# starlingonearth/MASt3R-SLAM-Quality-dualTSDF

Measured on AMD Instinct MI355X. Metric: SLAM frames/sec (infer+match+TSDF+GN) @512x384, higher is better.
Workload: dtype bf16

## Files before the change

include/mslam_hip.h:

```cpp
#ifndef MSLAM_HIP_H
#define MSLAM_HIP_H

#include <stddef.h>
#include <stdint.h>

#ifdef __cplusplus
extern "C" {
#endif

#define MSLAM_OK 0
#define MSLAM_EINVAL (-1)
#define MSLAM_EHIP (-2)
#define MSLAM_ENOMEM (-3)
#define MSLAM_ENODEV (-4)

const char* mslam_last_error(void);
int mslam_abi_version(void);
int mslam_device_check(void);


int mslam_iter_proj(const float* rays_img_with_grad, const float* pts_3d_norm,
                    const float* p_init, float* p_new, uint8_t* converged, int b, int h, int w,
                    int n, int max_iter, float lambda_init, float cost_thresh, void* stream);

int mslam_refine_matches(const uint16_t* D11, const uint16_t* D21, const int64_t* p1,
                         int64_t* p1_new, int b, int h, int w, int n, int fdim, int radius,
                         int dilation_max, void* stream);

int mslam_prep_iter_proj(const float* X11, const float* X21, const int64_t* idx_init,
                         float* rays_img_with_grad, float* pts_3d_norm, float* p_init, int b, int h,
                         int w, void* stream);

int mslam_match_occlusion(const float* X11, const float* X21, const float* p, int64_t* p1,
                          uint8_t* valid, int b, int h, int w, float dist_thresh, void* stream);

int mslam_pixel_to_lin(const int64_t* p1, int64_t* idx, int b, int n, int w, void* stream);

size_t mslam_gn_workspace_bytes(int num_poses, int num_edges, int num_points, int local_edges);

int mslam_gauss_newton_rays(float* Twc, const float* Xs, const float* Cs, const int64_t* ii,
                            const int64_t* jj, const int64_t* idx_ii2jj, const uint8_t* valid_match,
                            const float* Q, int num_poses, int num_points, int num_edges,
                            float sigma_ray, float sigma_dist, float C_thresh, float Q_thresh,
                            int max_iter, float delta_thresh, float* dx, void* workspace,
                            size_t workspace_bytes, void* stream);

int mslam_gauss_newton_calib(float* Twc, const float* Xs, const float* Cs, const float* K,
                             const int64_t* ii, const int64_t* jj, const int64_t* idx_ii2jj,
                             const uint8_t* valid_match, const float* Q, int num_poses, int num_points,
                             int num_edges, int height, int width, int pixel_border, float z_eps,
                             float sigma_pixel, float sigma_depth, float C_thresh, float Q_thresh,
                             int max_iter, float delta_thresh, float* dx, void* workspace,
                             size_t workspace_bytes, void* stream);

int mslam_gauss_newton_points(float* Twc, const float* Xs, const float* Cs, const int64_t* ii,
                              const int64_t* jj, const int64_t* idx_ii2jj, const uint8_t* valid_match,
                              const float* Q, int num_poses, int num_points, int num_edges,
                              float sigma_point, float C_thresh, float Q_thresh, int max_iter,
                              float delta_thresh, float* dx, void* workspace, size_t workspace_bytes,
                              void* stream);

int mslam_gn_begin(const int64_t* ii, const int64_t* jj, int num_poses, int num_edges, int num_points,
                   void* workspace, size_t workspace_bytes, void* stream);
int mslam_gn_compact(const float* Xs, const float* Cs, const int64_t* idx_ii2jj, const uint8_t* valid_match,
                     const float* Q, int num_poses, int num_points, int num_edges, int edge_begin,
                     int edge_count, float C_thresh, float Q_thresh, void* workspace, size_t workspace_bytes,
                     void* stream);
int mslam_gn_compact_at(const float* Xs, const float* Cs, const int64_t* idx_ii2jj, const uint8_t* valid_match,
                        const float* Q, int num_poses, int num_points, int num_edges, int edge_begin, int edge_count,
                        int slot_begin, int range_count, float C_thresh, float Q_thresh, void* workspace,
                        size_t workspace_bytes, void* stream);
int mslam_gn_accumulate(int kind, const float* Twc, const float* K, int num_poses, int num_points,
                        int num_edges, int edge_begin, int edge_count, float sigma_a, float sigma_b,
                        int height, int width, int pixel_border, float z_eps, float* Hs, float* gs,
                        void* workspace, size_t workspace_bytes, void* stream);
int mslam_gn_solve_retract(const float* Hs, const float* gs, int num_poses, int num_edges,
                           int num_points, float* Twc, float* dx, float delta_thresh, void* workspace,
                           size_t workspace_bytes, void* stream);
int mslam_gn_status(int* status4, int num_poses, int num_edges, int num_points, void* workspace,
                    size_t workspace_bytes, void* stream);

int mslam_sim3_act(const float* T, const float* X, float* Y, int num_poses, long long pts_per_pose,
                   int broadcast_pose, void* stream);
int mslam_sim3_op(int op, const float* A, const float* B, float* out, int n, int bcast_a, int bcast_b,
                  void* stream);

size_t mslam_tsdf_table_bytes(uint64_t capacity);
int mslam_tsdf_table_init(void* table, size_t table_bytes, uint64_t capacity, void* stream);

size_t mslam_tsdf_integrate_workspace_bytes(int n_points, double voxel_size, double trunc, double step_scale);
int mslam_tsdf_integrate(void* table, uint64_t capacity, const float* points_world, const double* conf,
                         const float* cam_origin, int n_points, double voxel_size, double trunc,
                         double max_weight, double step_scale, int shard_id, int num_shards,
                         void* workspace, size_t workspace_bytes, void* stream);

int mslam_tsdf_rehash(void* old_table, uint64_t old_capacity, void* new_table, uint64_t new_capacity, void* stream);
int mslam_tsdf_header(void* table, uint64_t capacity, uint32_t* out8_host, void* stream);

int mslam_tsdf_dump(void* table, uint64_t capacity, int64_t* keys, double* tsdf, double* weight,
                    uint32_t max_out, void* stream);

int mslam_tsdf_query(void* table, uint64_t capacity, const float* points, int n, double voxel_size,
                     double min_weight, double* value, double* grad, uint8_t* status, void* stream);

int mslam_tsdf_pose_step(void* table, uint64_t capacity, const float* points, const float* conf, int n,
                         float* pose, int points_in_camera_frame, double voxel_size, double min_weight,
                         double lambda, double damping, int update_pose, double* H_out, double* b_out,
                         int* used_out, void* workspace, size_t workspace_bytes, void* stream);

int mslam_tsdf_lookup7(void* table, uint64_t capacity, const float* points, int n, const float* pose,
                       double voxel_size, double* out, void* stream);
int mslam_tsdf_query_lookup(const double* lookup, int n, double voxel_size, double min_weight, double* value,
                            double* grad, uint8_t* status, void* stream);
int mslam_tsdf_pose_step_lookup(const double* lookup, const float* points, const float* conf, int n, float* pose,
                                int points_in_camera_frame, double voxel_size, double min_weight, double lambda,
                                double damping, int update_pose, double* H_out, double* b_out, int* used_out,
                                void* workspace, size_t workspace_bytes, void* stream);

size_t mslam_tsdf_mesh_workspace_bytes(uint64_t capacity);
int mslam_tsdf_mesh_keys(void* table, uint64_t capacity, double min_weight, int64_t* sort_keys, void* stream);
int mslam_tsdf_mesh_count(void* table, uint64_t capacity, double min_weight, double level, const int64_t* sorted_keys,
                          const int64_t* order, int32_t* counts, void* workspace, size_t workspace_bytes, void* stream);
int mslam_tsdf_mesh_emit(void* table, uint64_t capacity, double voxel_size, double min_weight, double level,
                         const int64_t* sorted_keys, const int64_t* order, const int64_t* vbase, const int64_t* fbase,
                         void* workspace, size_t workspace_bytes, float* vertices, float* normals, int32_t* faces,
                         int64_t n_vertices, int64_t n_faces, void* stream);
int mslam_tsdf_load(void* table, uint64_t capacity, const int64_t* keys, const double* tsdf, const double* weight,
                    int n, void* stream);

size_t mslam_tsdf_render_workspace_bytes(uint64_t capacity);
int mslam_tsdf_render_blocks(void* table, uint64_t capacity, double min_weight, void* workspace, size_t workspace_bytes,
                             void* stream);
int mslam_tsdf_render(void* table, uint64_t capacity, const float* rays, int h, int w, const float* pose8,
                      double voxel_size, double min_weight, double level, double near, double far, double step, int skip,
                      const void* workspace, size_t workspace_bytes, float* range, float* normal, uint8_t* hit,
                      void* stream);

size_t mslam_tsdf_color_bytes(uint64_t capacity);
int mslam_tsdf_color_init(void* color, size_t color_bytes, uint64_t capacity, void* stream);
int mslam_tsdf_integrate_color(void* table, uint64_t capacity, void* color, const float* points_world,
                               const double* conf, const float* rgb, const float* cam_origin, int n_points,
                               double voxel_size, double trunc, double step_scale, void* stream);
int mslam_tsdf_color_rehash(void* old_table, uint64_t old_capacity, const void* old_color, void* new_table,
                            uint64_t new_capacity, void* new_color, void* stream);
int mslam_tsdf_color_dump(void* table, uint64_t capacity, const void* color, const int64_t* keys, int n, uint64_t* sums,
                          void* stream);
int mslam_tsdf_color_load(void* table, uint64_t capacity, void* color, const int64_t* keys, const uint64_t* sums, int n,
                          void* stream);
int mslam_tsdf_color_sample(void* table, uint64_t capacity, const void* color, const float* points, int n, int image_w,
                            double voxel_size, double default_r, double default_g, double default_b, float* out_rgb,
                            uint8_t* out_count, void* stream);

int mslam_mast3r_create(void** handle_out, const int* cfg9_host, void* const* weight_ptrs_host,
                        const long long* weight_numels_host, int n_weights, void* stream);
int mslam_mast3r_destroy(void* handle);
size_t mslam_mast3r_workspace_bytes(void* handle, int batch, int H, int W);

int mslam_mast3r_encode(void* handle, const float* img, int batch, int H, int W, float* feat_out,
                        void* workspace, size_t workspace_bytes, void* stream);

int mslam_mast3r_decode(void* handle, const float* feat1, const float* feat2, int batch, int H, int W,
                        float* X1, float* C1, float* D1, float* Q1, float* X2, float* C2, float* D2,
                        float* Q2, float* dec_last1, float* dec_last2, void* workspace,
                        size_t workspace_bytes, void* stream);

size_t mslam_track_workspace_bytes(int n_points);
int mslam_track_pose(int use_calib, float* T_rel, const float* Xf, const float* Xk, const int64_t* idx_f2k,
                     const float* Qk, const uint8_t* valid, int n_points, const float* K, int width,
                     int height, float sigma_a, float sigma_b, float huber, int pixel_border, float z_eps,
                     int first_iter, int max_iters, float rel_error, float delta_norm, void* status_out, void* workspace,
                     size_t workspace_bytes, void* stream);

size_t mslam_track_prepare_workspace_bytes(int n_points);
int mslam_track_prepare(const int64_t* idx_f2k, const uint8_t* valid_match, const float* Qff, const float* Qkf,
                        const float* Cf_sum, float inv_nf, const float* Ck_sum, float inv_nk, float C_conf, float Q_conf,
                        int n_points, const float* T_WCk, const float* T_WCf, float* Qk, float* Ck_avg,
                        uint8_t* valid_opt, uint8_t* valid_kf, float* T_rel, void* workspace, size_t workspace_bytes,
                        void* stream);
int mslam_track_verdict(const void* prepare_workspace, const void* status, int n_points, float* verdict6, void* stream);
int mslam_track_fuse(const float* T_WCk, const float* T_rel, const float* Xkf, const float* Ckf, const float* X_canon,
                     const float* C, int n_points, float* T_WCf, float* X_new, float* C_new, void* stream);

int mslam_gemm_bf16(const void* A, const void* W, const float* bias, const void* residual_f32, void* out,
                    int M, int N, int K, int act, int out_is_bf16, void* stream);
int mslam_gemm_tile_override(int M, int N, int K, int cfg);
int mslam_gemm_profile_begin(int M, int N, int K, int max_samples);
int mslam_gemm_profile_end(double* avg_us, double* min_us, int* samples);
int mslam_conv2d_nhwc_bf16(const void* in, const void* W, const float* bias, const void* residual_bf16,
                           void* out_bf16, int B, int H, int Wd, int Cin, int Cout, int ks, int stride,
                           int relu_in, int act, void* stream);
int mslam_attention_bf16(const void* Q, const void* K, const void* VT, void* O, int batch, int heads,
                         int nq, int nk, void* stream);
int mslam_layernorm_f32(const float* x, const float* w, const float* b, void* out_bf16, float* out_f32,
                        int rows, int D, float eps, void* stream);

size_t mslam_tsdf_local_workspace_bytes(int n_points);
int mslam_tsdf_local_build(const float* X_world, const float* C, const float* origin, const float* xyz_min,
                           const float* xyz_max, int n_points, int nx, int ny, int nz, double voxel_size,
                           double trunc, float min_confidence, float* tsdf, float* weights, void* workspace,
                           size_t workspace_bytes, void* stream);
int mslam_tsdf_local_raycast(const float* tsdf, int nx, int ny, int nz, const float* xyz_min,
                             const float* xyz_max, const float* X_original, const int64_t* sel_pix, int n_sel,
                             int n_samples, float max_displacement, float* surf, uint8_t* hit, void* stream);

int mslam_quality_reduce_grid(const float* x, const float* y, const uint8_t* valid, int h, int w, int ps, int mode,
                              double c_thr, double q_thr, float* out, void* stream);
int mslam_quality_classify(const float* delta_cov, const float* r, const float* u, int n, float thr_zr, float thr_zu,
                           float thr_dc, int64_t* cls, float* pri, void* stream);

int mslam_room_pair(const float* ki, const float* kj, int batch, int h, int w, int n_frames, double fx, double fy,
                    double cx, double cy, double noise, const double* Wm_3x24, const double* phase_24, float* X1,
                    float* C1, float* D1, float* Q1, float* X2, float* C2, float* D2, float* Q2, void* stream);

int mslam_remap_bilinear_u8(const uint8_t* src, int src_h, int src_w, int channels, const float* mapx,
                            const float* mapy, uint8_t* dst, int dst_h, int dst_w, void* stream);

int mslam_gemm_f64(const void* A, int a_is_f32, const void* B, int b_is_f32, int b_transposed, const double* centre,
                   const double* bias, double* out, int M, int N, int K, void* stream);

int mslam_asmk_aggregate(const float* des, const float* centroids, const int64_t* assign, const int64_t* uniq_words,
                         uint32_t* sig_out, int n_des, int m_assign, int dim, int n_uniq, int n_centroids, void* stream);
int mslam_asmk_search(const int32_t* entry_word, const uint32_t* entry_sig, const int32_t* img_start, int n_images,
                      const int32_t* q_words, const uint32_t* q_sig, int n_q, int sig_words, float similarity_threshold,
                      float alpha, double* scores, void* stream);

#ifdef __cplusplus
}
#endif
#endif
```

mast3r-slam-quality-dualtsdf_amd/csrc/gemm.h:

```cpp
#pragma once
#include <hip/hip_runtime.h>
#include <stdint.h>

namespace mslam {

typedef __bf16 bf16;

enum GemmAct { ACT_NONE = 0, ACT_GELU = 1, ACT_RELU = 2 };
enum GemmKind { KIND_NONE = 0, KIND_F32 = 1, KIND_BF16 = 2 };
enum GemmEpi {
  EPI_PLAIN = 0,
  EPI_ATTN = 1,
  EPI_CONVT = 2,
};

struct GemmArgs {
  const bf16* A;
  const bf16* W;
  int M, N, K;
  int lda;
  int a_conv, cB, cH, cW, cC, cKs, cStride, cPad, cHo, cWo;
  int a_relu;
  const float* bias;
  int act;
  const void* res1; int res1_kind; int ldr1;
  const void* res2; int res2_kind; int ldr2;
  void* out; int out_kind; int ldc;
  int epi;
  bf16* q_out; bf16* k_out; bf16* vt_out;
  int sec_base;
  int sec_dim;
  int heads;
  int ntok;
  int tok_w;
  int kv_ntok;
  const float* rope_cos; const float* rope_sin;
  float q_scale;
  int ct_s, ct_cout, ct_h, ct_w;
  int groups;
  const bf16* W1; const float* bias1;
  size_t a_gstride;
  size_t out_gbytes, res1_gbytes, res2_gbytes;
  size_t qkv_gstride;
  const void* pf_ptr[2]; size_t pf_bytes[2];
  unsigned* pf_sink;
};

constexpr int kGemmPrefetchBlocks = 64;

int launch_gemm(const GemmArgs& a, hipStream_t stream);
int gemm_profile_begin(int M, int N, int K, int max_samples);
int gemm_profile_end(double* avg_us, double* min_us, int* samples);
int gemm_tile_override(int M, int N, int K, int cfg, bool conv);

}
```

mast3r-slam-quality-dualtsdf_amd/csrc/gemm.hip:

```cpp
#include <stdlib.h>
#include <mutex>
#include <unordered_map>
#include <vector>
#include "common.h"
#include "gemm.h"

namespace mslam {

int launch_gemm_t64(const GemmArgs& a, int stages, hipStream_t s);
int launch_gemm_t128(const GemmArgs& a, int waves, int stages, hipStream_t s);
int launch_gemm_t128x64(const GemmArgs& a, int stages, hipStream_t s);
int launch_gemm_t256(const GemmArgs& a, int bn, hipStream_t s);
int launch_gemm_t192(const GemmArgs& a, hipStream_t s);
int launch_gemm_t256w8(const GemmArgs& a, hipStream_t s);
int launch_gemm_8p(const GemmArgs& a, hipStream_t s);
bool gemm8p_supports(const GemmArgs& a);

static std::mutex g_tile_mu;
static inline uint64_t tile_key(int M, int N, int K, bool conv = false) {
  return (uint64_t)M | ((uint64_t)N << 22) | ((uint64_t)K << 42) | ((uint64_t)conv << 63);
}
static std::unordered_map<uint64_t, int> g_tile_override = {
    {tile_key(3072, 3072, 1024), 1262},
    {tile_key(3072, 768, 3072), 643},
    {tile_key(6144, 3072, 768), 1282},
    {tile_key(3072, 4096, 1024), 2192},
    {tile_key(6144, 4096, 1024), 1282},
    {tile_key(9216, 4096, 1024), 1282},
    {tile_key(9216, 1024, 4096), 8256},
    {tile_key(4608, 4096, 1024), 1282},
};

int gemm_tile_override(int M, int N, int K, int cfg, bool conv) {
  std::lock_guard<std::mutex> lk(g_tile_mu);
  if (cfg > 0) g_tile_override[tile_key(M, N, K, conv)] = cfg;
  else g_tile_override.erase(tile_key(M, N, K, conv));
  return 0;
}

static std::mutex g_prof_mu;
static struct {
  bool on = false;
  int M = 0, N = 0, K = 0, cap = 0, n = 0;
  std::vector<hipEvent_t> ev;
} g_prof;

int gemm_profile_begin(int M, int N, int K, int max_samples) {
  std::lock_guard<std::mutex> lk(g_prof_mu);
  MSLAM_REQUIRE(!g_prof.on, "gemm_profile_begin: already profiling");
  MSLAM_REQUIRE(max_samples > 0 && max_samples <= 65536, "gemm_profile_begin: max_samples out of range");
  g_prof.ev.resize(2 * (size_t)max_samples);
  for (auto& e : g_prof.ev) {
    int rc = check_hip(hipEventCreate(&e), "hipEventCreate");
    if (rc) return rc;
  }
  g_prof.M = M; g_prof.N = N; g_prof.K = K; g_prof.cap = max_samples; g_prof.n = 0;
  g_prof.on = true;
  return MSLAM_OK;
}

int gemm_profile_end(double* avg_us, double* min_us, int* samples) {
  std::lock_guard<std::mutex> lk(g_prof_mu);
  MSLAM_REQUIRE(g_prof.on, "gemm_profile_end: not profiling");
  g_prof.on = false;
  double sum = 0.0, mn = 1e30;
  int rc = MSLAM_OK;
  for (int i = 0; i < g_prof.n && !rc; i++) {
    float ms = 0.0f;
    rc = check_hip(hipEventSynchronize(g_prof.ev[2 * i + 1]), "hipEventSynchronize");
    if (!rc) rc = check_hip(hipEventElapsedTime(&ms, g_prof.ev[2 * i], g_prof.ev[2 * i + 1]), "hipEventElapsedTime");
    sum += 1e3 * ms;
    if (1e3 * ms < mn) mn = 1e3 * ms;
  }
  if (samples) *samples = g_prof.n;
  if (avg_us) *avg_us = g_prof.n ? sum / g_prof.n : 0.0;
  if (min_us) *min_us = g_prof.n ? mn : 0.0;
  for (auto& e : g_prof.ev) (void)hipEventDestroy(e);
  g_prof.ev.clear();
  return rc;
}

static int launch_gemm_impl(const GemmArgs& a, hipStream_t stream);

int launch_gemm(const GemmArgs& a, hipStream_t stream) {
  int slot = -1;
  if (g_prof.on) {
    std::lock_guard<std::mutex> lk(g_prof_mu);
    if (g_prof.on && !a.a_conv && a.groups <= 1 && a.M == g_prof.M && a.N == g_prof.N && a.K == g_prof.K &&
        g_prof.n < g_prof.cap) {
      slot = g_prof.n++;
      (void)hipEventRecord(g_prof.ev[2 * slot], stream);
    }
  }
  const int rc = launch_gemm_impl(a, stream);
  if (slot >= 0) (void)hipEventRecord(g_prof.ev[2 * slot + 1], stream);
  return rc;
}

static int launch_gemm_impl(const GemmArgs& a, hipStream_t stream) {
  MSLAM_REQUIRE(a.M > 0 && a.N > 0 && a.K > 0, "gemm: empty problem %dx%dx%d", a.M, a.N, a.K);
  MSLAM_REQUIRE(a.K % 8 == 0, "gemm: K=%d must be a multiple of 8", a.K);
  MSLAM_REQUIRE(!a.a_conv || a.cC % 8 == 0, "gemm: conv channels %d must be a multiple of 8", a.cC);
  MSLAM_REQUIRE(a.a_conv || a.lda % 8 == 0, "gemm: lda=%d must be a multiple of 8", a.lda);
  MSLAM_REQUIRE(!a.a_relu || a.a_conv, "gemm: ReLU-on-load is only built for the implicit-conv view");
  MSLAM_REQUIRE(((uintptr_t)a.A & 15) == 0 && ((uintptr_t)a.W & 15) == 0, "gemm: A and W must be 16-byte aligned");
  const size_t a_bytes = a.a_conv ? (size_t)a.cB * a.cH * a.cW * a.cC * 2 : ((size_t)(a.M - 1) * a.lda + a.K) * 2;
  MSLAM_REQUIRE(a_bytes < (1ull << 31) && (size_t)a.N * a.K * 2 < (1ull << 31), "gemm: operand larger than 2 GiB");
  MSLAM_REQUIRE(a.epi != EPI_ATTN || (a.sec_dim % 64 == 0 && a.ntok % 4 == 0 && a.kv_ntok % 4 == 0),
                "gemm: attention epilogue needs 64-wide heads and token counts divisible by 4");
  static int forced = -2;
  if (forced == -2) {
    const char* e = getenv("MSLAM_GEMM");
    forced = e ? atoi(e) : -1;
  }
  MSLAM_REQUIRE(a.groups <= 2 && (a.groups < 2 || (a.W1 && !a.a_conv)), "gemm: bad group description");
  const long ngrp = a.groups > 1 ? 2 : 1;
  auto blocks = [&](int bm, int bn) { return ngrp * ((a.M + bm - 1) / bm) * ((a.N + bn - 1) / bn); };
  int cfg = forced;
  if (cfg < 0 && a.groups <= 1 && a.M < (1 << 22) && a.N < (1 << 20) && a.K < (1 << 20)) {
    static const bool log_shapes = getenv("MSLAM_GEMM_LOG") != nullptr;
    static std::unordered_map<uint64_t, int> seen;
    std::lock_guard<std::mutex> lk(g_tile_mu);
    const uint64_t key = tile_key(a.M, a.N, a.K, a.a_conv != 0);
    auto it = g_tile_override.find(key);
    if (it != g_tile_override.end()) cfg = it->second;
    if (log_shapes && seen.emplace(key, 1).second) fprintf(stderr, "mslam_gemm_shape conv=%d %d %d %d\n", (int)(a.a_conv != 0), a.M, a.N, a.K);
  }
  if (cfg < 0) {
    const bool narrow = a.N <= 128 || (a.N > 256 && a.N <= 384);
    if (narrow && blocks(256, 128) >= 128) cfg = 2128;
    else if (blocks(256, 256) >= 128) cfg = 2256;
    else if (blocks(128, 128) >= 256) cfg = 1282;
    else if (blocks(64, 64) >= 512) cfg = 642;
    else if (a.K >= 2048) cfg = 644;
    else cfg = 643;
  }
  switch (cfg) {
    case 642: return launch_gemm_t64(a, 2, stream);
    case 643: return launch_gemm_t64(a, 3, stream);
    case 644: return launch_gemm_t64(a, 4, stream);
    case 1262: return launch_gemm_t128x64(a, 2, stream);
    case 1263: return launch_gemm_t128x64(a, 3, stream);
    case 1242: return launch_gemm_t128(a, 4, 2, stream);
    case 1282: return launch_gemm_t128(a, 8, 2, stream);
    case 1283: return launch_gemm_t128(a, 8, 3, stream);
    case 2128: return launch_gemm_t256(a, 128, stream);
    case 2256: return launch_gemm_t256(a, 256, stream);
    case 2192: return launch_gemm_t192(a, stream);
    case 2258: return launch_gemm_t256w8(a, stream);
    case 8256: return gemm8p_supports(a) ? launch_gemm_8p(a, stream) : launch_gemm_t256(a, 256, stream);
    default: MSLAM_REQUIRE(false, "gemm: unknown configuration %d", cfg);
  }
}

}
```

mast3r-slam-quality-dualtsdf_amd/csrc/mast3r.hip:

```cpp
#include <stdlib.h>
#include <vector>
#include "common.h"
#include "gemm.h"

namespace mslam {

int launch_attention(const bf16* Q, const bf16* K, const bf16* VT, bf16* O, int batch, int heads, int nq, int nk,
                     hipStream_t stream);

template <typename TIN>
__global__ __launch_bounds__(256) void layernorm_kernel(const TIN* __restrict__ x, const float* __restrict__ w,
                                                        const float* __restrict__ b, bf16* __restrict__ out_bf,
                                                        float* __restrict__ out_f, int rows, int D, float eps) {
  constexpr int MAXV = 32;
  const int row = blockIdx.x * 4 + (threadIdx.x >> 6);
  const int lane = threadIdx.x & 63;
  if (row >= rows) return;
  const TIN* xr = x + (size_t)row * D;
  float v[MAXV];
  float s = 0.0f;
#pragma unroll
  for (int c = 0; c < MAXV; c++) {
    const int i = lane + 64 * c;
    v[c] = (i < D) ? (float)xr[i] : 0.0f;
// ... 557 lines not shown
}

static bf16* rcu(Ctx& c, const bf16* x, int B, int H, int W, int C, const Rcu& r, const bf16* extra) {
  bf16* t = conv(c, x, B, H, W, C, r.c1, 3, 1,  1, ACT_RELU, nullptr, nullptr);
  return conv(c, t, B, H, W, C, r.c2, 3, 1, 0, ACT_NONE, x, extra);
}

static bf16* fusion(Ctx& c, const Fusion& f, const bf16* path, const bf16* layer, int B, int H, int W, int C) {
  const bf16* s = path;
  if (f.has_r1) s = rcu(c, layer, B, H, W, C, f.r1, path);
  bf16* r = rcu(c, s, B, H, W, C, f.r2, nullptr);
  bf16* o = conv(c, r, B, H, W, C, f.out, 1, 1, 0, ACT_NONE, nullptr, nullptr);
  return upsample2x(c, o, B, H, W, C);
}

struct HeadOut { float *X, *C, *D, *Q; };

static void run_head(Ctx& c, const Head& hd, const bf16* const toks[4], int B, int H, int W, const HeadOut& out) {
  const Mast3rModel& m = *c.m;
  const int nh = H / m.P, nw = W / m.P, M = B * nh * nw;
  bf16* t0 = conv(c, toks[0], B, nh, nw, m.E, hd.a00, 1, 1, 0, ACT_NONE, nullptr, nullptr);
  bf16* l0 = conv_transpose(c, t0, B, nh, nw, hd.a00.out, hd.a01, 4, hd.a00.out);
  bf16* t1 = conv(c, toks[1], B, nh, nw, m.Dd, hd.a10, 1, 1, 0, ACT_NONE, nullptr, nullptr);
  bf16* l1 = conv_transpose(c, t1, B, nh, nw, hd.a10.out, hd.a11, 2, hd.a10.out);
  bf16* l2 = conv(c, toks[2], B, nh, nw, m.Dd, hd.a20, 1, 1, 0, ACT_NONE, nullptr, nullptr);
  bf16* t3 = conv(c, toks[3], B, nh, nw, m.Dd, hd.a30, 1, 1, 0, ACT_NONE, nullptr, nullptr);
  bf16* l3 = conv(c, t3, B, nh, nw, hd.a30.out, hd.a31, 3, 2, 0, ACT_NONE, nullptr, nullptr);
  const int h3 = (nh + 2 - 3) / 2 + 1, w3 = (nw + 2 - 3) / 2 + 1;
  bf16* r0 = conv(c, l0, B, 4 * nh, 4 * nw, hd.a00.out, hd.rn[0], 3, 1, 0, ACT_NONE, nullptr, nullptr);
  bf16* r1 = conv(c, l1, B, 2 * nh, 2 * nw, hd.a10.out, hd.rn[1], 3, 1, 0, ACT_NONE, nullptr, nullptr);
  bf16* r2 = conv(c, l2, B, nh, nw, hd.a20.out, hd.rn[2], 3, 1, 0, ACT_NONE, nullptr, nullptr);
  bf16* r3 = conv(c, l3, B, h3, w3, hd.a30.out, hd.rn[3], 3, 1, 0, ACT_NONE, nullptr, nullptr);
  if (2 * h3 != nh || 2 * w3 != nw) {
    if (!c.dry()) set_error("mast3r head: token grid %dx%d must be even", nh, nw);
    c.fail(MSLAM_EINVAL);
    return;
  }
  const int fd = m.fd;
  bf16* p4 = fusion(c, hd.fus[3], r3, nullptr, B, h3, w3, fd);
  bf16* p3 = fusion(c, hd.fus[2], p4, r2, B, nh, nw, fd);
  bf16* p2 = fusion(c, hd.fus[1], p3, r1, B, 2 * nh, 2 * nw, fd);
  bf16* p1 = fusion(c, hd.fus[0], p2, r0, B, 4 * nh, 4 * nw, fd);
  bf16* h0 = conv(c, p1, B, 8 * nh, 8 * nw, fd, hd.h0, 3, 1, 0, ACT_NONE, nullptr, nullptr);
  bf16* hu = upsample2x(c, h0, B, 8 * nh, 8 * nw, hd.h0.out);
  bf16* h2 = conv(c, hu, B, H, W, hd.h0.out, hd.h2, 3, 1, 0, ACT_RELU, nullptr, nullptr);
  const int idim = m.E + m.Dd;
  bf16* cat = c.ar.get<bf16>((size_t)M * idim);
  bf16* hid = c.ar.get<bf16>((size_t)M * hd.fc1.out);
  float* lf = c.ar.get<float>((size_t)M * hd.fc2.out);
  if (!c.dry() && !c.rc) {
    const size_t total = (size_t)M * idim;
    hipLaunchKernelGGL(concat2_kernel, dim3((unsigned)((total + 255) / 256)), dim3(256), 0, c.s, toks[0], m.E, toks[3],
                       m.Dd, cat, (size_t)M);
    dbg(c, "concat2", M);
  }
  linear_bf16(c, cat, M, hd.fc1, hid, ACT_GELU);
  linear_f32(c, hid, M, hd.fc2, lf);
  if (!c.dry() && !c.rc) {
    if (m.P == kHP && hd.h2.out == 128 && m.desc_dim == 24) {
      hipLaunchKernelGGL(head_post_kernel, dim3((unsigned)(B * (H / m.P) * (W / m.P))), dim3(256), 0, c.s, h2, hd.h2.out,
                         hd.h4w, hd.h4b, lf, hd.fc2.out, m.desc_dim, B, H, W, out.X, out.C, out.D, out.Q);
    } else {
      const size_t npix = (size_t)B * H * W;
      hipLaunchKernelGGL(head_post_generic_kernel, dim3((unsigned)((npix + 255) / 256)), dim3(256), 0, c.s, h2, hd.h2.out,
                         hd.h4w, hd.h4b, lf, hd.fc2.out, m.desc_dim, m.P, B, H, W, out.X, out.C, out.D, out.Q);
    }
    dbg(c, "head_post", B, H, W);
  }
}

static void g_layernorm(Ctx& c, const float* x, const Norm& n0, const Norm& n1, int M, bf16* out) {
  if (c.dry() || c.rc) return;
  const LnSet s0{n0.w, n0.b}, s1{n1.w, n1.b};
  const dim3 grid((2 * M + 3) / 4), block(256);
  if (n0.d == 768) hipLaunchKernelGGL((layernorm_group_vec_kernel<3, false>), grid, block, 0, c.s, x, s0, s1, s0, s1, out, out, M, 1e-6f);
  else if (n0.d == 1024) hipLaunchKernelGGL((layernorm_group_vec_kernel<4, false>), grid, block, 0, c.s, x, s0, s1, s0, s1, out, out, M, 1e-6f);
  else {
    launch_layernorm(x, n0.w, n0.b, out, nullptr, M, n0.d, 1e-6f, c.s);
    launch_layernorm(x + (size_t)M * n0.d, n1.w, n1.b, out + (size_t)M * n0.d, nullptr, M, n0.d, 1e-6f, c.s);
  }
  dbg(c, "g_layernorm", M, n0.d);
}

static void g_layernorm_cross(Ctx& c, const float* x, const DecBlock& b0, const DecBlock& b1, int M, bf16* h, bf16* yn) {
  if (c.dry() || c.rc) return;
  const int D = b0.n1.d;
  const dim3 grid((2 * M + 3) / 4), block(256);
  const LnSet self0{b0.n1.w, b0.n1.b}, self1{b1.n1.w, b1.n1.b}, mem0{b0.ny.w, b0.ny.b}, mem1{b1.ny.w, b1.ny.b};
  if (D == 768) hipLaunchKernelGGL((layernorm_group_vec_kernel<3, true>), grid, block, 0, c.s, x, self0, self1, mem0, mem1, h, yn, M, 1e-6f);
  else if (D == 1024) hipLaunchKernelGGL((layernorm_group_vec_kernel<4, true>), grid, block, 0, c.s, x, self0, self1, mem0, mem1, h, yn, M, 1e-6f);
  else {
    const size_t MD = (size_t)M * D;
    launch_layernorm(x, b0.n1.w, b0.n1.b, h, nullptr, M, D, 1e-6f, c.s);
    launch_layernorm(x + MD, b1.n1.w, b1.n1.b, h + MD, nullptr, M, D, 1e-6f, c.s);
    launch_layernorm(x + MD, b0.ny.w, b0.ny.b, yn, nullptr, M, D, 1e-6f, c.s);
    launch_layernorm(x, b1.ny.w, b1.ny.b, yn + MD, nullptr, M, D, 1e-6f, c.s);
  }
  dbg(c, "g_layernorm_cross", M, D);
}

static void dec_layer_grouped(Ctx& c, const DecBlock& b0, const DecBlock& b1, const DecBlock* n0, const DecBlock* n1,
                              float* x, bf16* yn, int B, int N, int nw, BlockScratch& s) {
  const Mast3rModel& m = *c.m;
  const int M = B * N;
  const auto pf = [&](Lin DecBlock::*f) { return n0 ? Pf{&(n0->*f), &(n1->*f)} : Pf{}; };
  g_layernorm_cross(c, x, b0, b1, M, s.h, yn);
  attn_project(c, s.h, M, b0.qkv, 0, m.dec_heads, N, N, nw, s.ab, pf(&DecBlock::qkv), &b1.qkv);
  attention(c, s.ab, 2 * B, m.dec_heads, N, N);
  linear_residual(c, s.ab.o, M, b0.proj, x, pf(&DecBlock::proj), &b1.proj);
  g_layernorm(c, x, b0.n2, b1.n2, M, s.h);
  attn_project(c, s.h, M, b0.pq, 0, m.dec_heads, N, N, nw, s.ab, pf(&DecBlock::pq), &b1.pq);
  attn_project(c, yn, M, b0.pkv, 1, m.dec_heads, N, N, nw, s.ab, pf(&DecBlock::pkv), &b1.pkv);
  attention(c, s.ab, 2 * B, m.dec_heads, N, N);
  linear_residual(c, s.ab.o, M, b0.cproj, x, pf(&DecBlock::cproj), &b1.cproj);
  g_layernorm(c, x, b0.n3, b1.n3, M, s.h);
  linear_bf16(c, s.h, M, b0.fc1, s.u, ACT_GELU, pf(&DecBlock::fc1), &b1.fc1);
  linear_residual(c, s.u, M, b0.fc2, x, pf(&DecBlock::fc2), &b1.fc2);
}

static void decode(Ctx& c, const float* feat1, const float* feat2, int B, int H, int W, const HeadOut out[2],
                   float* dec_last1, float* dec_last2) {
  const Mast3rModel& m = *c.m;
  const int nh = H / m.P, nw = W / m.P, N = nh * nw, M = B * N;
  float* dec_last[2] = {dec_last1, dec_last2};
  const size_t ME = (size_t)M * m.E, MD = (size_t)M * m.Dd;
  bf16* fb_all = c.ar.get<bf16>(2 * ME);
  float* x_all = c.ar.get<float>(2 * MD);
  bf16* yn_all = c.ar.get<bf16>(2 * MD);
  bf16* tok_all[4] = {fb_all, c.ar.get<bf16>(2 * MD), c.ar.get<bf16>(2 * MD), c.ar.get<bf16>(2 * MD)};
  BlockScratch bs_all = block_scratch(c, 2 * M, m.Dd);
  cast_bf16(c, feat1, fb_all, ME);
  cast_bf16(c, feat2, c.dry() ? nullptr : fb_all + ME, ME);
  linear_f32(c, fb_all, 2 * M, m.dec_embed, x_all);
  for (int l = 0; l < m.dec_depth; l++) {
    const bool more = l + 1 < m.dec_depth;
    dec_layer_grouped(c, m.dec[0][l], m.dec[1][l], more ? &m.dec[0][l + 1] : nullptr, more ? &m.dec[1][l + 1] : nullptr,
                      x_all, yn_all, B, N, nw, bs_all);
    for (int k = 1; k < 3; k++)
      if (l + 1 == m.hooks[k]) cast_bf16(c, x_all, tok_all[k], 2 * MD);
  }
  const size_t mark = c.ar.off;
  for (int s = 0; s < 2; s++) {
    bf16* tok[4];
    for (int k = 0; k < 4; k++) tok[k] = c.dry() ? nullptr : tok_all[k] + s * (k ? MD : ME);
    layernorm(c, c.dry() ? nullptr : x_all + s * MD, m.dec_norm, M, tok[3], dec_last[s]);
    c.ar.off = mark;
    run_head(c, m.head[s], tok, B, H, W, out[s]);
  }
}

}

using namespace mslam;

extern "C" int mslam_mast3r_create(void** handle_out, const int* cfg9, void* const* weight_ptrs,
                                   const long long* weight_numels, int n_weights, void* stream) {
  MSLAM_REQUIRE(handle_out && cfg9 && weight_ptrs && weight_numels, "mast3r_create: null pointer");
  Mast3rModel* m = new Mast3rModel();
  m->E = cfg9[0]; m->enc_depth = cfg9[1]; m->enc_heads = cfg9[2]; m->Dd = cfg9[3]; m->dec_depth = cfg9[4];
  m->dec_heads = cfg9[5]; m->P = cfg9[6]; m->desc_dim = cfg9[7]; m->fd = cfg9[8];
  if (m->E != m->enc_heads * 64 || m->Dd != m->dec_heads * 64 || m->desc_dim > 31 || m->P < 1 || m->fd % 8) {
    set_error("mast3r_create: head_dim must be 64 (enc %d/%d, dec %d/%d), desc_dim <= 31", m->E, m->enc_heads, m->Dd,
              m->dec_heads);
    delete m;
    return MSLAM_EINVAL;
  }
  const int l2 = m->dec_depth;
  m->hooks[0] = 0; m->hooks[1] = l2 * 2 / 4; m->hooks[2] = l2 * 3 / 4; m->hooks[3] = l2;
  PtrFeed f{weight_ptrs, weight_numels, n_weights};
  const int E = m->E, D = m->Dd, P = m->P;
  m->pe = f.lin(E, 3 * P * P, true, "patch_embed");
  for (int i = 0; i < m->enc_depth; i++) {
    EncBlock b;
    b.n1 = f.norm(E, "enc.norm1"); b.qkv = f.lin(3 * E, E, true, "enc.qkv"); b.proj = f.lin(E, E, true, "enc.proj");
    b.n2 = f.norm(E, "enc.norm2"); b.fc1 = f.lin(4 * E, E, true, "enc.fc1"); b.fc2 = f.lin(E, 4 * E, true, "enc.fc2");
    m->enc.push_back(b);
  }
  m->enc_norm = f.norm(E, "enc_norm");
  m->dec_embed = f.lin(D, E, true, "decoder_embed");
  for (int s = 0; s < 2; s++)
    for (int i = 0; i < m->dec_depth; i++) {
      DecBlock b;
      b.n1 = f.norm(D, "dec.norm1"); b.qkv = f.lin(3 * D, D, true, "dec.qkv"); b.proj = f.lin(D, D, true, "dec.proj");
      b.n2 = f.norm(D, "dec.norm2"); b.ny = f.norm(D, "dec.norm_y");
      b.pq = f.lin(D, D, true, "dec.projq"); b.pkv = f.lin(2 * D, D, true, "dec.projkv");
      b.cproj = f.lin(D, D, true, "dec.cross_proj");
      b.n3 = f.norm(D, "dec.norm3"); b.fc1 = f.lin(4 * D, D, true, "dec.fc1"); b.fc2 = f.lin(D, 4 * D, true, "dec.fc2");
      m->dec[s].push_back(b);
    }
  m->dec_norm = f.norm(D, "dec_norm");
  const int dims[4] = {96, 192, 384, 768};
  const int fd = m->fd;
  for (int s = 0; s < 2; s++) {
    Head& h = m->head[s];
    h.a00 = f.lin(dims[0], E, true, "act0.0"); h.a01 = f.lin(dims[0] * 16, dims[0], false, "act0.1");
    h.a01.b = (const float*)f.take(dims[0], "act0.1.bias");
    h.a10 = f.lin(dims[1], D, true, "act1.0"); h.a11 = f.lin(dims[1] * 4, dims[1], false, "act1.1");
    h.a11.b = (const float*)f.take(dims[1], "act1.1.bias");
    h.a20 = f.lin(dims[2], D, true, "act2.0");
    h.a30 = f.lin(dims[3], D, true, "act3.0"); h.a31 = f.lin(dims[3], 9 * dims[3], true, "act3.1");
    for (int k = 0; k < 4; k++) h.rn[k] = f.lin(fd, 9 * dims[k], false, "layer_rn");
    for (int k = 3; k >= 0; k--) {
      Fusion& fu = h.fus[k];
      fu.has_r1 = (k != 3);
      if (fu.has_r1) { fu.r1.c1 = f.lin(fd, 9 * fd, true, "rcu1.conv1"); fu.r1.c2 = f.lin(fd, 9 * fd, true, "rcu1.conv2"); }
      fu.r2.c1 = f.lin(fd, 9 * fd, true, "rcu2.conv1"); fu.r2.c2 = f.lin(fd, 9 * fd, true, "rcu2.conv2");
      fu.out = f.lin(fd, fd, true, "out_conv");
    }
    h.h0 = f.lin(fd / 2, 9 * fd, true, "head.0"); h.h2 = f.lin(fd / 2, 9 * (fd / 2), true, "head.2");
    h.h4w = (const float*)f.take(4 * (fd / 2), "head.4.weight"); h.h4b = (const float*)f.take(4, "head.4.bias");
    const int idim = E + D;
    h.fc1 = f.lin(4 * idim, idim, true, "lf.fc1"); h.fc2 = f.lin((m->desc_dim + 1) * P * P, 4 * idim, true, "lf.fc2");
  }
  if (!f.ok) { delete m; return MSLAM_EINVAL; }
  if (f.pos != n_weights) {
    set_error("mast3r_create: %d weights supplied, %d consumed", n_weights, f.pos);
    delete m;
    return MSLAM_EINVAL;
  }
  m->rope_len = 1024;
  std::vector<float> hc((size_t)m->rope_len * 16), hs((size_t)m->rope_len * 16);
  for (int p = 0; p < m->rope_len; p++)
    for (int i = 0; i < 16; i++) {
      const float inv_freq = 1.0f / powf(100.0f, (float)(2 * i) / 32.0f);
      const float fr = (float)p * inv_freq;
      hc[(size_t)p * 16 + i] = cosf(fr);
      hs[(size_t)p * 16 + i] = sinf(fr);
    }
  int rc = check_hip(hipMalloc(&m->rope_cos, hc.size() * 4 + 16), "rope hipMalloc");
  if (!rc) m->pf_sink = reinterpret_cast<unsigned*>(m->rope_cos + hc.size());
  if (!rc) rc = check_hip(hipMalloc(&m->rope_sin, hs.size() * 4), "rope hipMalloc");
  if (!rc) rc = check_hip(hipMemcpyAsync(m->rope_cos, hc.data(), hc.size() * 4, hipMemcpyHostToDevice, (hipStream_t)stream), "rope copy");
  if (!rc) rc = check_hip(hipMemcpyAsync(m->rope_sin, hs.data(), hs.size() * 4, hipMemcpyHostToDevice, (hipStream_t)stream), "rope copy");
  if (!rc) rc = check_hip(hipStreamSynchronize((hipStream_t)stream), "rope sync");
  if (const char* e = getenv("MSLAM_PREFETCH")) m->prefetch = atoi(e) != 0;
  if (rc) { delete m; return rc; }
  *handle_out = m;
  return MSLAM_OK;
}

extern "C" int mslam_mast3r_destroy(void* handle) {
  Mast3rModel* m = (Mast3rModel*)handle;
  if (!m) return MSLAM_OK;
  if (m->rope_cos) (void)hipFree(m->rope_cos);
  if (m->rope_sin) (void)hipFree(m->rope_sin);
  delete m;
  return MSLAM_OK;
}

static int check_shape(const Mast3rModel* m, int B, int H, int W, const char* who) {
  MSLAM_REQUIRE(m, "%s: null model", who);
  MSLAM_REQUIRE(B >= 1 && H >= m->P && W >= m->P && H % m->P == 0 && W % m->P == 0,
                "%s: image %dx%d must be a positive multiple of the patch size %d", who, H, W, m->P);
  const int N = (H / m->P) * (W / m->P);
  MSLAM_REQUIRE(N % 8 == 0, "%s: token count %d must be a multiple of 8", who, N);
  MSLAM_REQUIRE(m->E <= 2048 && m->Dd <= 2048, "%s: embedding dims above 2048 unsupported", who);
  MSLAM_REQUIRE(H / m->P < m->rope_len && W / m->P < m->rope_len, "%s: token grid exceeds the RoPE table", who);
  return MSLAM_OK;
}

extern "C" size_t mslam_mast3r_workspace_bytes(void* handle, int batch, int H, int W) {
  const Mast3rModel* m = (const Mast3rModel*)handle;
  if (!m || check_shape(m, batch, H, W, "mast3r_workspace_bytes")) return 0;
  Ctx c{m, Arena{nullptr, 0, 0, true}, nullptr};
  encode(c, nullptr, batch, H, W, nullptr);
  c.ar.off = 0;
  HeadOut out[2] = {};
  decode(c, nullptr, nullptr, batch, H, W, out, nullptr, nullptr);
  return c.ar.peak + 4096;
}

extern "C" int mslam_mast3r_encode(void* handle, const float* img, int batch, int H, int W, float* feat_out,
                                   void* workspace, size_t workspace_bytes, void* stream) {
  const Mast3rModel* m = (const Mast3rModel*)handle;
  int rc = check_shape(m, batch, H, W, "mast3r_encode");
  if (rc) return rc;
  MSLAM_REQUIRE(img && feat_out && workspace, "mast3r_encode: null pointer");
  MSLAM_REQUIRE(workspace_bytes >= mslam_mast3r_workspace_bytes(handle, batch, H, W), "mast3r_encode: workspace too small");
  Ctx c{m, Arena{(char*)workspace, 0, workspace_bytes, false}, (hipStream_t)stream};
  encode(c, img, batch, H, W, feat_out);
  MSLAM_REQUIRE(!c.ar.overflow, "mast3r_encode: workspace arena overflow (%zu > %zu)", c.ar.peak, c.ar.cap);
  if (c.rc) return c.rc;
  return check_hip(hipGetLastError(), "mast3r_encode launch");
}

extern "C" int mslam_mast3r_decode(void* handle, const float* feat1, const float* feat2, int batch, int H, int W,
                                   float* X1, float* C1, float* D1, float* Q1, float* X2, float* C2, float* D2,
                                   float* Q2, float* dec_last1, float* dec_last2, void* workspace,
                                   size_t workspace_bytes, void* stream) {
  const Mast3rModel* m = (const Mast3rModel*)handle;
  int rc = check_shape(m, batch, H, W, "mast3r_decode");
  if (rc) return rc;
  MSLAM_REQUIRE(feat1 && feat2 && X1 && C1 && D1 && Q1 && X2 && C2 && D2 && Q2 && workspace, "mast3r_decode: null pointer");
  MSLAM_REQUIRE(workspace_bytes >= mslam_mast3r_workspace_bytes(handle, batch, H, W), "mast3r_decode: workspace too small");
  Ctx c{m, Arena{(char*)workspace, 0, workspace_bytes, false}, (hipStream_t)stream};
  HeadOut out[2] = {{X1, C1, D1, Q1}, {X2, C2, D2, Q2}};
  decode(c, feat1, feat2, batch, H, W, out, dec_last1, dec_last2);
  MSLAM_REQUIRE(!c.ar.overflow, "mast3r_decode: workspace arena overflow (%zu > %zu)", c.ar.peak, c.ar.cap);
  if (c.rc) return c.rc;
  return check_hip(hipGetLastError(), "mast3r_decode launch");
}

extern "C" int mslam_gemm_tile_override(int M, int N, int K, int cfg) {
  MSLAM_REQUIRE(M != 0 && N > 0 && K > 0 && cfg >= 0, "gemm_tile_override: bad arguments");
  return gemm_tile_override(M < 0 ? -M : M, N, K, cfg, M < 0);
}

extern "C" int mslam_gemm_profile_begin(int M, int N, int K, int max_samples) {
  return gemm_profile_begin(M, N, K, max_samples);
}

extern "C" int mslam_gemm_profile_end(double* avg_us, double* min_us, int* samples) {
  return gemm_profile_end(avg_us, min_us, samples);
}

extern "C" int mslam_gemm_bf16(const void* A, const void* Wt, const float* bias, const void* residual_f32, void* out,
                               int M, int N, int K, int act, int out_is_bf16, void* stream) {
  MSLAM_REQUIRE(A && Wt && out, "gemm_bf16: null pointer");
  GemmArgs g = {};
  g.A = (const bf16*)A; g.W = (const bf16*)Wt; g.M = M; g.N = N; g.K = K; g.lda = K; g.bias = bias; g.act = act;
  g.out = out; g.out_kind = out_is_bf16 ? KIND_BF16 : KIND_F32; g.ldc = N; g.ldr1 = N; g.ldr2 = N;
  if (residual_f32) { g.res1 = residual_f32; g.res1_kind = KIND_F32; }
  return launch_gemm(g, (hipStream_t)stream);
}

extern "C" int mslam_conv2d_nhwc_bf16(const void* in, const void* Wt, const float* bias, const void* residual_bf16,
                                      void* out_bf16, int B, int H, int Wd, int Cin, int Cout, int ks, int stride,
                                      int relu_in, int act, void* stream) {
  MSLAM_REQUIRE(in && Wt && out_bf16, "conv2d: null pointer");
  MSLAM_REQUIRE((ks == 1 || ks == 3) && (stride == 1 || stride == 2), "conv2d: unsupported ks/stride");
  Lin l; l.W = (const bf16*)Wt; l.b = bias; l.out = Cout; l.in = ks * ks * Cin;
  GemmArgs g = conv_args((const bf16*)in, B, H, Wd, Cin, l, ks, stride);
  g.out = out_bf16; g.a_relu = relu_in; g.act = act;
  if (residual_bf16) { g.res1 = residual_bf16; g.res1_kind = KIND_BF16; }
  return launch_gemm(g, (hipStream_t)stream);
}

extern "C" int mslam_attention_bf16(const void* Q, const void* K, const void* VT, void* O, int batch, int heads,
                                    int nq, int nk, void* stream) {
  MSLAM_REQUIRE(Q && K && VT && O, "attention: null pointer");
  return launch_attention((const bf16*)Q, (const bf16*)K, (const bf16*)VT, (bf16*)O, batch, heads, nq, nk,
                          (hipStream_t)stream);
}

extern "C" int mslam_layernorm_f32(const float* x, const float* w, const float* b, void* out_bf16, float* out_f32,
                                   int rows, int D, float eps, void* stream) {
  MSLAM_REQUIRE(x && w && b && (out_bf16 || out_f32), "layernorm: null pointer");
  MSLAM_REQUIRE(D <= 2048 && rows > 0, "layernorm: D=%d must be <= 2048", D);
  launch_layernorm(x, w, b, (bf16*)out_bf16, out_f32, rows, D, eps, (hipStream_t)stream);
  MSLAM_LAUNCH_CHECK("layernorm");
  return MSLAM_OK;
}
```

Measured before the change: 163.6.

## Replace GEMM tile heuristics with cost-model-based tile selection

Replaces the threshold-based GEMM tile selection with an analytic cost model. The model estimates runtime per tile config from tile count, CU residency, wave quantization, per-MAC throughput and epilogue cost, and it also covers grouped GEMMs. Most hand-tuned shape overrides are removed and one grouped override is added, with the override key extended by a grouped bit. It also exposes a grouped GEMM C entry point and a config query API. The risk is that the hardcoded cost constants pick worse tiles than the old overrides for some shapes.

```diff
diff --git a/include/mslam_hip.h b/include/mslam_hip.h
--- a/include/mslam_hip.h
+++ b/include/mslam_hip.h
@@ -184,6 +184,9 @@
 int mslam_gemm_bf16(const void* A, const void* W, const float* bias, const void* residual_f32, void* out,
                     int M, int N, int K, int act, int out_is_bf16, void* stream);
 int mslam_gemm_tile_override(int M, int N, int K, int cfg);
+int mslam_gemm_choose_cfg(int M, int N, int K, int groups, int conv, int heavy_epilogue, int allow_8p);
+int mslam_gemm_bf16_grouped(const void* A, const void* W0, const void* W1, const float* bias0, const float* bias1,
+                            void* out, int M, int N, int K, int act, void* stream);
 int mslam_gemm_profile_begin(int M, int N, int K, int max_samples);
 int mslam_gemm_profile_end(double* avg_us, double* min_us, int* samples);
 int mslam_conv2d_nhwc_bf16(const void* in, const void* W, const float* bias, const void* residual_bf16,
diff --git a/mast3r-slam-quality-dualtsdf_amd/csrc/gemm.h b/mast3r-slam-quality-dualtsdf_amd/csrc/gemm.h
--- a/mast3r-slam-quality-dualtsdf_amd/csrc/gemm.h
+++ b/mast3r-slam-quality-dualtsdf_amd/csrc/gemm.h
@@ -51,6 +51,7 @@
 int launch_gemm(const GemmArgs& a, hipStream_t stream);
 int gemm_profile_begin(int M, int N, int K, int max_samples);
 int gemm_profile_end(double* avg_us, double* min_us, int* samples);
-int gemm_tile_override(int M, int N, int K, int cfg, bool conv);
+int gemm_tile_override(int M, int N, int K, int cfg, bool conv, bool grouped);
+int gemm_choose_cfg(int M, int N, int K, int groups, int conv, int heavy_epi, int can_8p);
 
 }
diff --git a/mast3r-slam-quality-dualtsdf_amd/csrc/gemm.hip b/mast3r-slam-quality-dualtsdf_amd/csrc/gemm.hip
--- a/mast3r-slam-quality-dualtsdf_amd/csrc/gemm.hip
+++ b/mast3r-slam-quality-dualtsdf_amd/csrc/gemm.hip
@@ -17,24 +17,20 @@
 bool gemm8p_supports(const GemmArgs& a);
 
 static std::mutex g_tile_mu;
-static inline uint64_t tile_key(int M, int N, int K, bool conv = false) {
-  return (uint64_t)M | ((uint64_t)N << 22) | ((uint64_t)K << 42) | ((uint64_t)conv << 63);
+static inline uint64_t tile_key(int M, int N, int K, bool conv = false, bool grouped = false) {
+  return (uint64_t)M | ((uint64_t)N << 22) | ((uint64_t)K << 42) | ((uint64_t)grouped << 62) | ((uint64_t)conv << 63);
 }
 static std::unordered_map<uint64_t, int> g_tile_override = {
     {tile_key(3072, 3072, 1024), 1262},
     {tile_key(3072, 768, 3072), 643},
     {tile_key(6144, 3072, 768), 1282},
-    {tile_key(3072, 4096, 1024), 2192},
-    {tile_key(6144, 4096, 1024), 1282},
-    {tile_key(9216, 4096, 1024), 1282},
-    {tile_key(9216, 1024, 4096), 8256},
-    {tile_key(4608, 4096, 1024), 1282},
+    {tile_key(1536, 3072, 768, false, true), 1262},
 };
 
-int gemm_tile_override(int M, int N, int K, int cfg, bool conv) {
+int gemm_tile_override(int M, int N, int K, int cfg, bool conv, bool grouped) {
   std::lock_guard<std::mutex> lk(g_tile_mu);
-  if (cfg > 0) g_tile_override[tile_key(M, N, K, conv)] = cfg;
-  else g_tile_override.erase(tile_key(M, N, K, conv));
+  if (cfg > 0) g_tile_override[tile_key(M, N, K, conv, grouped)] = cfg;
+  else g_tile_override.erase(tile_key(M, N, K, conv, grouped));
   return 0;
 }
 
@@ -78,6 +74,75 @@
   for (auto& e : g_prof.ev) (void)hipEventDestroy(e);
   g_prof.ev.clear();
   return rc;
+}
+
+struct TileCost {
+  int cfg, bm, bn, resident;
+  float fix_us, epi_us, us_per_mmac, alone_us_per_mmac;
+  bool needs_company;
+};
+static constexpr TileCost kTileCost[] = {
+    {2256, 256, 256, 1, 10.4f, 7.2f, 0.265f, 0.265f, false},
+    {8256, 256, 256, 1, 12.5f, 7.3f, 0.236f, 0.236f, false},
+    {2192, 192, 256, 1, 9.5f, 6.0f, 0.333f, 0.333f, false},
+    {2128, 256, 128, 1, 7.6f, 2.5f, 0.379f, 0.379f, false},
+    {1282, 128, 128, 2, 5.2f, 1.8f, 0.386f, 0.544f, false},
+    {1262, 128, 64, 3, 3.6f, 1.8f, 0.540f, 0.553f, true},
+    {643, 64, 64, 3, 2.4f, 0.0f, 0.714f, 0.867f, false},
+};
+
+static int device_cus() {
+  static const int cus = [] {
+    int dev = 0;
+    hipDeviceProp_t p;
+    if (hipGetDevice(&dev) != hipSuccess || hipGetDeviceProperties(&p, dev) != hipSuccess || p.multiProcessorCount <= 0) {
+      (void)hipGetLastError();
+      return 256;
+    }
+    return p.multiProcessorCount;
+  }();
+  return cus;
+}
+
+static double tile_cost_us(const TileCost& t, long M, long N, long K, long ngrp, bool heavy_epi, int cus) {
+  const long tiles = ngrp * ((M + t.bm - 1) / t.bm) * ((N + t.bn - 1) / t.bn);
+  const long slots = (long)cus * t.resident, full = tiles / slots, rem = tiles % slots;
+  const long last = (rem + cus - 1) / cus;
+  const double mmac = 1e-6 * t.bm * t.bn * (double)K;
+  double us = (double)(full + (rem ? 1 : 0)) * (t.fix_us + (heavy_epi ? t.epi_us : 0.0f));
+  us += mmac * (double)(full * t.resident) * t.us_per_mmac;
+  us += mmac * (double)last * (last == t.resident ? t.us_per_mmac : t.alone_us_per_mmac);
+  return us;
+}
+
+static int gemm_rule_cfg(long M, long N, long K, long ngrp, bool heavy_epi, bool can_8p) {
+  const int cus = device_cus();
+  int best = 0;
+  double best_us = 0.0;
+  for (const TileCost& t : kTileCost) {
+    if (t.cfg == 8256 && !can_8p) continue;
+    if (t.needs_company && ngrp * ((M + t.bm - 1) / t.bm) * ((N + t.bn - 1) / t.bn) <= cus) continue;
+    const double us = tile_cost_us(t, M, N, K, ngrp, heavy_epi, cus);
+    if (!best || us < best_us) { best = t.cfg; best_us = us; }
+  }
+  if (best == 643) {
+    const long tiles = ngrp * ((M + 63) / 64) * ((N + 63) / 64);
+    if (tiles >= 2L * cus) best = 642;
+    else if (K >= 2048) best = 644;
+  }
+  return best;
+}
+
+static bool tile_key_fits(long M, long N, long K) { return M < (1 << 22) && N < (1 << 20) && K < (1 << 20); }
+
+int gemm_choose_cfg(int M, int N, int K, int groups, int conv, int heavy_epi, int can_8p) {
+  const bool grouped = groups > 1;
+  if (tile_key_fits(M, N, K)) {
+    std::lock_guard<std::mutex> lk(g_tile_mu);
+    auto it = g_tile_override.find(tile_key(M, N, K, conv != 0, grouped));
+    if (it != g_tile_override.end() && (it->second != 8256 || can_8p)) return it->second;
+  }
+  return gemm_rule_cfg(M, N, K, grouped ? 2 : 1, heavy_epi != 0, can_8p != 0);
 }
 
 static int launch_gemm_impl(const GemmArgs& a, hipStream_t stream);
@@ -114,26 +179,17 @@
     forced = e ? atoi(e) : -1;
   }
   MSLAM_REQUIRE(a.groups <= 2 && (a.groups < 2 || (a.W1 && !a.a_conv)), "gemm: bad group description");
-  const long ngrp = a.groups > 1 ? 2 : 1;
-  auto blocks = [&](int bm, int bn) { return ngrp * ((a.M + bm - 1) / bm) * ((a.N + bn - 1) / bn); };
   int cfg = forced;
-  if (cfg < 0 && a.groups <= 1 && a.M < (1 << 22) && a.N < (1 << 20) && a.K < (1 << 20)) {
+  if (cfg < 0) {
+    cfg = gemm_choose_cfg(a.M, a.N, a.K, a.groups, a.a_conv != 0, a.act == ACT_GELU || a.epi == EPI_ATTN, gemm8p_supports(a));
     static const bool log_shapes = getenv("MSLAM_GEMM_LOG") != nullptr;
-    static std::unordered_map<uint64_t, int> seen;
-    std::lock_guard<std::mutex> lk(g_tile_mu);
-    const uint64_t key = tile_key(a.M, a.N, a.K, a.a_conv != 0);
-    auto it = g_tile_override.find(key);
-    if (it != g_tile_override.end()) cfg = it->second;
-    if (log_shapes && seen.emplace(key, 1).second) fprintf(stderr, "mslam_gemm_shape conv=%d %d %d %d\n", (int)(a.a_conv != 0), a.M, a.N, a.K);
-  }
-  if (cfg < 0) {
-    const bool narrow = a.N <= 128 || (a.N > 256 && a.N <= 384);
-    if (narrow && blocks(256, 128) >= 128) cfg = 2128;
-    else if (blocks(256, 256) >= 128) cfg = 2256;
-    else if (blocks(128, 128) >= 256) cfg = 1282;
-    else if (blocks(64, 64) >= 512) cfg = 642;
-    else if (a.K >= 2048) cfg = 644;
-    else cfg = 643;
+    if (log_shapes && tile_key_fits(a.M, a.N, a.K)) {
+      static std::unordered_map<uint64_t, int> seen;
+      std::lock_guard<std::mutex> lk(g_tile_mu);
+      if (seen.emplace(tile_key(a.M, a.N, a.K, a.a_conv != 0, a.groups > 1), 1).second)
+        fprintf(stderr, "mslam_gemm_shape conv=%d groups=%d %d %d %d act=%d epi=%d cfg=%d\n", (int)(a.a_conv != 0),
+                a.groups > 1 ? 2 : 1, a.M, a.N, a.K, a.act, a.epi, cfg);
+    }
   }
   switch (cfg) {
     case 642: return launch_gemm_t64(a, 2, stream);
diff --git a/mast3r-slam-quality-dualtsdf_amd/csrc/mast3r.hip b/mast3r-slam-quality-dualtsdf_amd/csrc/mast3r.hip
--- a/mast3r-slam-quality-dualtsdf_amd/csrc/mast3r.hip
+++ b/mast3r-slam-quality-dualtsdf_amd/csrc/mast3r.hip
@@ -883,8 +883,13 @@
 }
 
 extern "C" int mslam_gemm_tile_override(int M, int N, int K, int cfg) {
-  MSLAM_REQUIRE(M != 0 && N > 0 && K > 0 && cfg >= 0, "gemm_tile_override: bad arguments");
-  return gemm_tile_override(M < 0 ? -M : M, N, K, cfg, M < 0);
+  MSLAM_REQUIRE(M != 0 && N != 0 && (M > 0 || N > 0) && K > 0 && cfg >= 0, "gemm_tile_override: bad arguments");
+  return gemm_tile_override(M < 0 ? -M : M, N < 0 ? -N : N, K, cfg, M < 0, N < 0);
+}
+
+extern "C" int mslam_gemm_choose_cfg(int M, int N, int K, int groups, int conv, int heavy_epilogue, int allow_8p) {
+  if (M <= 0 || N <= 0 || K <= 0 || groups < 1 || groups > 2 || (conv && groups > 1)) return 0;
+  return gemm_choose_cfg(M, N, K, groups, conv, heavy_epilogue, allow_8p && groups == 1 && !conv);
 }
 
 extern "C" int mslam_gemm_profile_begin(int M, int N, int K, int max_samples) {
@@ -902,6 +907,18 @@
   g.A = (const bf16*)A; g.W = (const bf16*)Wt; g.M = M; g.N = N; g.K = K; g.lda = K; g.bias = bias; g.act = act;
   g.out = out; g.out_kind = out_is_bf16 ? KIND_BF16 : KIND_F32; g.ldc = N; g.ldr1 = N; g.ldr2 = N;
   if (residual_f32) { g.res1 = residual_f32; g.res1_kind = KIND_F32; }
+  return launch_gemm(g, (hipStream_t)stream);
+}
+
+extern "C" int mslam_gemm_bf16_grouped(const void* A, const void* W0, const void* W1, const float* bias0,
+                                       const float* bias1, void* out, int M, int N, int K, int act, void* stream) {
+  MSLAM_REQUIRE(A && W0 && W1 && out, "gemm_bf16_grouped: null pointer");
+  MSLAM_REQUIRE(M > 0 && N > 0 && K > 0, "gemm_bf16_grouped: empty problem %dx%dx%d", M, N, K);
+  GemmArgs g = {};
+  g.A = (const bf16*)A; g.W = (const bf16*)W0; g.M = M; g.N = N; g.K = K; g.lda = K; g.bias = bias0; g.act = act;
+  g.out = out; g.out_kind = KIND_BF16; g.ldc = N; g.ldr1 = N; g.ldr2 = N;
+  g.groups = 2; g.W1 = (const bf16*)W1; g.bias1 = bias1; g.a_gstride = (size_t)M * K;
+  g.out_gbytes = (size_t)M * N * sizeof(bf16);
   return launch_gemm(g, (hipStream_t)stream);
 }
 
```

New measurement: 163.7, median of 2. Within noise of the previous version (+0.0%).
